# yukara-ikemiya/friendly-stable-audio-tools

Hardware: NVIDIA H100
Metric: denoise_steps_per_s (higher is better)
Workload: dtype fp16 operands, fp32 accumulate (the reference's autocast dtype)

## Files before the change

friendly-stable-audio-tools_b200/csrc/attention_tc.cu:

```cuda
#include "common.cuh"
#include "gemm.cuh"
#include "kernels.h"
#include "ptx.cuh"
#include <cmath>

namespace satb {

namespace {

constexpr int kQ = 64;
constexpr int kK = 64;
constexpr int kAttnThreads = 128;
template <int D>
constexpr int tile_elems() { return 64 * D; }
template <int D>
constexpr int attn_smem() { return (1 + 2 * 2) * tile_elems<D>() * 2; }

struct AttnArgs {
  const uint16_t *q, *k, *v;
  uint16_t* o;
  int64_t ldq, ldk, ldv, ldo, q_bs, k_bs, v_bs, o_bs;
  int q_col, k_col, v_col;
  int Nq, Nk, group;
  float scale_log2;
};

template <int D>
// ... 186 lines not shown
    l[i] += __shfl_xor_sync(0xffffffffu, l[i], 2);
    inv[i] = 1.f / l[i];
  }
  const int rr = warp * 16 + (lane >> 2);
#pragma unroll
  for (int j = 0; j < D / 8; ++j) {
    const int col = 8 * j + 2 * (lane & 3);
    *reinterpret_cast<uint32_t*>(sQ + swz<D>(rr, col >> 3) + (col & 7)) = Op16<BF16>::pack(o[j][0] * inv[0], o[j][1] * inv[0]);
    *reinterpret_cast<uint32_t*>(sQ + swz<D>(rr + 8, col >> 3) + (col & 7)) =
        Op16<BF16>::pack(o[j][2] * inv[1], o[j][3] * inv[1]);
  }
  __syncwarp();
  uint16_t* ob = p.o + b * p.o_bs + h * D;
#pragma unroll
  for (int i = 0; i < 16 * kChunks / 32; ++i) {
    const int idx = lane + 32 * i;
    const int r = warp * 16 + chunk_row<kChunks>(idx), c = chunk_col<kChunks>(idx);
    if (q0 + r < p.Nq)
      *reinterpret_cast<uint4*>(ob + static_cast<int64_t>(q0 + r) * p.ldo + c * 8) =
          *reinterpret_cast<const uint4*>(sQ + swz<D>(r, c));
  }
}

}

int launch_attention_tc(const void* q, const void* k, const void* v, void* o, int64_t ldq, int64_t ldk, int64_t ldv,
                        int64_t ldo, int64_t q_bs, int64_t k_bs, int64_t v_bs, int64_t o_bs, int q_cols, int k_cols,
                        int v_cols, int q_col, int k_col, int v_col, int batch, int H, int H_kv, int Nq, int Nk,
                        int head_dim, bool bf16, cudaStream_t stream) {
  SATB_REQUIRE(head_dim == 32 || head_dim == 64 || head_dim == 96 || head_dim == 128,
               "attention head dim must be 32, 64, 96 or 128");
  SATB_REQUIRE(H >= 1 && H_kv >= 1, "attention needs at least one head");
  SATB_REQUIRE(H % H_kv == 0, "num_heads must be a multiple of kv heads");
  SATB_REQUIRE(Nk >= 1 && Nq >= 1, "empty attention problem");
  SATB_REQUIRE(ldo % 8 == 0 && o_bs % 8 == 0 && (reinterpret_cast<uintptr_t>(o) & 15) == 0,
               "attention output must be 16B aligned");
  SATB_REQUIRE(ldq % 8 == 0 && ldk % 8 == 0 && ldv % 8 == 0 && q_col % 8 == 0 && k_col % 8 == 0 && v_col % 8 == 0 &&
                   q_bs % 8 == 0 && k_bs % 8 == 0 && v_bs % 8 == 0,
               "attention operand strides / column offsets must be 16B aligned");
  SATB_REQUIRE((reinterpret_cast<uintptr_t>(q) & 15) == 0 && (reinterpret_cast<uintptr_t>(k) & 15) == 0 &&
                   (reinterpret_cast<uintptr_t>(v) & 15) == 0,
               "attention operands must be 16B aligned");
  const int64_t dh = head_dim;
  SATB_REQUIRE(q_col + H * dh <= q_cols && k_col + H_kv * dh <= k_cols && v_col + H_kv * dh <= v_cols,
               "attention heads exceed the operand columns");
  AttnArgs a;
  a.q = static_cast<const uint16_t*>(q); a.k = static_cast<const uint16_t*>(k); a.v = static_cast<const uint16_t*>(v);
  a.o = static_cast<uint16_t*>(o);
  a.ldq = ldq; a.ldk = ldk; a.ldv = ldv; a.ldo = ldo;
  a.q_bs = q_bs; a.k_bs = k_bs; a.v_bs = v_bs; a.o_bs = o_bs;
  a.q_col = q_col; a.k_col = k_col; a.v_col = v_col;
  a.Nq = Nq; a.Nk = Nk; a.group = H / H_kv;
  a.scale_log2 = (1.0f / sqrtf(static_cast<float>(head_dim))) * 1.4426950408889634f;
  const dim3 grid(ceil_div(Nq, kQ), H, batch);
  SATB_REQUIRE(grid.y <= 65535 && grid.z <= 65535, "attention grid too large");
  auto go = [&](auto kern, int smem, PerDeviceOnce& once) -> int {
    if (once.first()) SATB_CHECK_CUDA(cudaFuncSetAttribute(kern, cudaFuncAttributeMaxDynamicSharedMemorySize, smem));
    SATB_CHECK_CUDA(launch_pdl(kern, grid, dim3(kAttnThreads), smem, stream, a));
    return 0;
  };
  static PerDeviceOnce once[4][2];
  PerDeviceOnce& on = once[head_dim / 32 - 1][bf16 ? 1 : 0];
  switch (head_dim) {
    case 32: SATB_PROPAGATE(bf16 ? go(attn_kernel<32, true>, attn_smem<32>(), on) : go(attn_kernel<32, false>, attn_smem<32>(), on)); break;
    case 64: SATB_PROPAGATE(bf16 ? go(attn_kernel<64, true>, attn_smem<64>(), on) : go(attn_kernel<64, false>, attn_smem<64>(), on)); break;
    case 96: SATB_PROPAGATE(bf16 ? go(attn_kernel<96, true>, attn_smem<96>(), on) : go(attn_kernel<96, false>, attn_smem<96>(), on)); break;
    default: SATB_PROPAGATE(bf16 ? go(attn_kernel<128, true>, attn_smem<128>(), on) : go(attn_kernel<128, false>, attn_smem<128>(), on)); break;
  }
  count_launch();
  SATB_CHECK_CUDA(cudaGetLastError());
  return 0;
}

}
```

friendly-stable-audio-tools_b200/csrc/dit.cu:

```cuda
#include <algorithm>
#include <cmath>
#include <cstring>
#include <map>
#include <string>
#include <tuple>
#include <vector>

#include "../../include/satb200.h"
#include "common.cuh"
#include "gemm.cuh"
#include "kernels.h"

namespace satb {

struct DevBuf {
  void* p = nullptr;
  size_t bytes = 0;
  int ensure(size_t need) {
    if (need <= bytes) return 0;
    if (p) cudaFree(p);
    p = nullptr;
    bytes = 0;
    cudaError_t e = cudaMalloc(&p, need);
    if (e != cudaSuccess) {
// ... 598 lines not shown
      SATB_PROPAGATE(launch_layernorm(h, W.pre_g, W.pre_b, a16, M, D, ssg_l, ssg_l ? ssg_l + D : nullptr, ssg_ld, N_seq, B, BF16, st));
    }
    {
      ProfScope ps(d, PROF_QKV, st);
      if (d->qk_norm) {
        typedef EpiHeadNorm16<BF16> E;
        typename E::Params ep{qkv, 3 * D, 2 * D, 2 * D, N_seq, cos_tab, sin_tab};
        SATB_PROPAGATE((linear<E, 256, BF16>(d->tmaps, a16, D, M, D, W.w_qkv, 3 * D, ep, st)));
      } else {
        if (fused && i > 0) {
          typedef EpiQkvRope<BF16, true> E;
          typename E::Params ep{qkv, 3 * D, 2 * D, N_seq, d->dh, d->nf, cos_tab, sin_tab, fold(S1, W.c_qkv, W.d_qkv)};
          SATB_PROPAGATE((linear<E, 256, BF16>(d->tmaps, a16, D, M, D, W.w_qkv, 3 * D, ep, st)));
        } else {
          typedef EpiQkvRope<BF16> E;
          typename E::Params ep{qkv, 3 * D, 2 * D, N_seq, d->dh, d->nf, cos_tab, sin_tab, no_ln};
          SATB_PROPAGATE((linear<E, 256, BF16>(d->tmaps, a16, D, M, D, W.w_qkv, 3 * D, ep, st)));
        }
      }
    }
    {
      ProfScope ps(d, PROF_ATTN_SELF, st);
      const int64_t qs = static_cast<int64_t>(N_seq) * 3 * D;
      SATB_PROPAGATE(launch_attention_tc(qkv, qkv, qkv, att, 3 * D, 3 * D, 3 * D, D, qs, qs, qs,
                                         static_cast<int64_t>(N_seq) * D, 3 * D, 3 * D, 3 * D, 0, D, 2 * D, R, H, H,
                                         N_seq, N_seq, d->dh, BF16, st));
    }
    {
      ProfScope ps(d, PROF_ATTN_OUT, st);
      if (fused) {
        typedef EpiResidualLN<BF16> E;
        typename E::Params ep{h, D, nullptr, a16, W.ca_g, W.ff_g, S2, S3, Mc};
        SATB_PROPAGATE((linear<E, 256, BF16>(d->tmaps, att, D, M, D, W.w_o, D, ep, st)));
      } else {
        EpiResidual::Params ep{h, D, nullptr, ssg_l ? ssg_l + 2 * D : nullptr, N_seq, static_cast<int>(ssg_ld), B};
        SATB_PROPAGATE((linear_auto<EpiResidual, BF16>(d->tmaps, att, D, M, D, W.w_o, D, ep, st)));
      }
    }
    if (Mc > 0) {
      ProfScope ps(d, PROF_CROSS, st);
      const int Hkv = d->ce / d->dh;
      if (!fused) SATB_PROPAGATE(launch_layernorm(h, W.ca_g, W.ca_b, a16, Mc, D, nullptr, nullptr, 0, N_seq, 1, BF16, st));
      if (d->qk_norm) {
        typedef EpiHeadNorm16<BF16> E;
        typename E::Params ep{q16, D, D, 0, N_seq, nullptr, nullptr};
        SATB_PROPAGATE((linear_auto<E, BF16>(d->tmaps, a16, D, Mc, D, W.w_q, D, ep, st)));
      } else {
        if (fused) {
          typedef EpiStore16<BF16, true> E;
          typename E::Params ep{q16, D, nullptr, 0, fold(S2, W.c_q, W.d_q)};
          SATB_PROPAGATE((linear_auto<E, BF16>(d->tmaps, a16, D, Mc, D, W.w_q, D, ep, st)));
        } else {
          typedef EpiStore16<BF16> E;
          typename E::Params ep{q16, D, nullptr, 0, no_ln};
          SATB_PROPAGATE((linear_auto<E, BF16>(d->tmaps, a16, D, Mc, D, W.w_q, D, ep, st)));
        }
      }
      const uint16_t* kv = d->ws_kv.as<uint16_t>() + static_cast<size_t>(i) * d->Rc * d->Mctx * 2 * d->ce;
      const int64_t kvs = static_cast<int64_t>(d->Mctx) * 2 * d->ce;
      SATB_PROPAGATE(launch_attention_tc(q16, kv, kv, att, D, 2 * d->ce, 2 * d->ce, D, static_cast<int64_t>(N_seq) * D,
                                         kvs, kvs, static_cast<int64_t>(N_seq) * D, D, 2 * d->ce, 2 * d->ce, 0, 0,
                                         d->ce, d->Rc, H, Hkv, N_seq, d->Mctx, d->dh, BF16, st));
      if (fused) {
        typedef EpiResidualLN<BF16> E;
        typename E::Params ep{h, D, nullptr, a16, W.ff_g, W.ff_g, S3, S3, Mc};
        SATB_PROPAGATE((linear<E, 256, BF16>(d->tmaps, att, D, Mc, D, W.w_co, D, ep, st)));
      } else {
        EpiResidual::Params ep{h, D, nullptr, nullptr, N_seq, 0, 1};
        SATB_PROPAGATE((linear_auto<EpiResidual, BF16>(d->tmaps, att, D, Mc, D, W.w_co, D, ep, st)));
      }
    }
    if (!fused) {
      ProfScope ps(d, PROF_LN, st);
      SATB_PROPAGATE(launch_layernorm(h, W.ff_g, W.ff_b, a16, M, D, ssg_l ? ssg_l + 3 * D : nullptr,
                                      ssg_l ? ssg_l + 4 * D : nullptr, ssg_ld, N_seq, B, BF16, st));
    }
    {
      ProfScope ps(d, PROF_FF_IN, st);
      if (fused) {
        typedef EpiSwiglu<BF16, true> E;
        typename E::Params ep{ff, d->ffi, W.b_ff1, fold(S3, W.c_ff1, W.d_ff1)};
        SATB_PROPAGATE((linear<E, 256, BF16>(d->tmaps, a16, D, M, D, W.w_ff1, 2 * d->ffi, ep, st)));
      } else {
        typedef EpiSwiglu<BF16> E;
        typename E::Params ep{ff, d->ffi, W.b_ff1, no_ln};
// ... 196 lines not shown
```

friendly-stable-audio-tools_b200/csrc/kernels.h:

```cpp
#pragma once
#include <cuda_runtime.h>
#include <stdint.h>

namespace satb {

int launch_attention_tc(const void* q, const void* k, const void* v, void* o, int64_t ldq, int64_t ldk, int64_t ldv,
                        int64_t ldo, int64_t q_bs, int64_t k_bs, int64_t v_bs, int64_t o_bs, int q_cols, int k_cols,
                        int v_cols, int q_col, int k_col, int v_col, int batch, int H, int H_kv, int Nq, int Nk,
                        int head_dim, bool bf16, cudaStream_t stream);
bool conv_halo_enabled();
bool resunit_use_fused();
bool conv_epi_masked();
bool ln_fold_enabled();
bool raw_stream_16bit();

int launch_layernorm(const float* x, const float* gamma, const float* beta, void* out16, int rows, int D,
                     const float* scale, const float* shift, int64_t mod_stride, int rows_per_item, int n_items,
                     bool bf16, cudaStream_t stream);
int launch_ln_fold_vectors(const void* w16, const float* gamma, const float* beta, float* c, float* d, int rows, int K,
                           bool bf16, cudaStream_t stream);
int launch_sampler_update(const float* x, const float* v, const float* d1, const float* d2, const float* nz, float* den,
                          float* x_next, float* x_in, long long n, float c_skip, float c_out, float A, float B, float C,
                          float D, float S, float c_in_next, cudaStream_t stream);
int launch_snake_beta(const float* x, const float* alpha, const float* beta, float* y, int B, int C, int64_t T,
                      int logscale, cudaStream_t stream);
int launch_dit_pre(const float* x, void* a16, int R, int B_src, int C, int L, int P, bool bf16, cudaStream_t stream);
int launch_fourier(const float* t, const float* w, float* out, int B, int F, cudaStream_t stream);
int launch_skinny_linear(const float* in, const float* W, const float* bias, const float* add, float* out, int R,
                         int K, int N, int silu_out, cudaStream_t stream);
int launch_write_prepend(const float* tok, const float* pre, float* h, int R, int B, int N_seq, int D, int Pp,
                         cudaStream_t stream);
int launch_gate_sigmoid(float* ssg, int rows, int depth, int D, cudaStream_t stream);
// ... 9 lines not shown
```

friendly-stable-audio-tools_b200/csrc/ptx.cuh:

```cuda
#pragma once
#include <cuda.h>
#include <cuda_runtime.h>
#include <stdint.h>

namespace satb {

__device__ __forceinline__ uint32_t smem_u32(const void* p) {
  return static_cast<uint32_t>(__cvta_generic_to_shared(p));
}

__device__ __forceinline__ bool elect_one() {
  uint32_t pred = 0;
  asm volatile(
      "{\n\t.reg .pred P;\n\t"
      "elect.sync _|P, 0xffffffff;\n\t"
      "selp.u32 %0, 1, 0, P;\n\t}"
      : "=r"(pred));
  return pred != 0;
}

__device__ __forceinline__ void pdl_wait() { asm volatile("griddepcontrol.wait;" ::: "memory"); }
__device__ __forceinline__ void pdl_launch_dependents() { asm volatile("griddepcontrol.launch_dependents;" ::: "memory"); }

__device__ __forceinline__ void mbar_init(uint64_t* bar, uint32_t count) {
// ... 142 lines not shown
template <>
__device__ __forceinline__ void wgmma_ss<256, false>(float (&d)[128], uint64_t da, uint64_t db, uint32_t accumulate) {
  asm volatile(
      "{\n\t.reg .pred p;\n\t"
      "setp.ne.b32 p, %130, 0;\n\t"
      "wgmma.mma_async.sync.aligned.m64n256k16.f32.f16.f16 "
      "{%0, %1, %2, %3, %4, %5, %6, %7, %8, %9, %10, %11, %12, %13, %14, %15, %16, %17, %18, %19, %20, %21, %22, %23, %24, %25, %26, %27, %28, %29, %30, %31, %32, %33, %34, %35, %36, %37, %38, %39, %40, %41, %42, %43, %44, %45, %46, %47, %48, %49, %50, %51, %52, %53, %54, %55, %56, %57, %58, %59, %60, %61, %62, %63, %64, %65, %66, %67, %68, %69, %70, %71, %72, %73, %74, %75, %76, %77, %78, %79, %80, %81, %82, %83, %84, %85, %86, %87, %88, %89, %90, %91, %92, %93, %94, %95, %96, %97, %98, %99, %100, %101, %102, %103, %104, %105, %106, %107, %108, %109, %110, %111, %112, %113, %114, %115, %116, %117, %118, %119, %120, %121, %122, %123, %124, %125, %126, %127}, "
      "%128, %129, p, 1, 1, 0, 0;\n\t}"
      : "+f"(d[0]), "+f"(d[1]), "+f"(d[2]), "+f"(d[3]), "+f"(d[4]), "+f"(d[5]), "+f"(d[6]), "+f"(d[7]), "+f"(d[8]), "+f"(d[9]), "+f"(d[10]), "+f"(d[11]), "+f"(d[12]), "+f"(d[13]), "+f"(d[14]), "+f"(d[15]), "+f"(d[16]), "+f"(d[17]), "+f"(d[18]), "+f"(d[19]), "+f"(d[20]), "+f"(d[21]), "+f"(d[22]), "+f"(d[23]), "+f"(d[24]), "+f"(d[25]), "+f"(d[26]), "+f"(d[27]), "+f"(d[28]), "+f"(d[29]), "+f"(d[30]), "+f"(d[31]), "+f"(d[32]), "+f"(d[33]), "+f"(d[34]), "+f"(d[35]), "+f"(d[36]), "+f"(d[37]), "+f"(d[38]), "+f"(d[39]), "+f"(d[40]), "+f"(d[41]), "+f"(d[42]), "+f"(d[43]), "+f"(d[44]), "+f"(d[45]), "+f"(d[46]), "+f"(d[47]), "+f"(d[48]), "+f"(d[49]), "+f"(d[50]), "+f"(d[51]), "+f"(d[52]), "+f"(d[53]), "+f"(d[54]), "+f"(d[55]), "+f"(d[56]), "+f"(d[57]), "+f"(d[58]), "+f"(d[59]), "+f"(d[60]), "+f"(d[61]), "+f"(d[62]), "+f"(d[63]), "+f"(d[64]), "+f"(d[65]), "+f"(d[66]), "+f"(d[67]), "+f"(d[68]), "+f"(d[69]), "+f"(d[70]), "+f"(d[71]), "+f"(d[72]), "+f"(d[73]), "+f"(d[74]), "+f"(d[75]), "+f"(d[76]), "+f"(d[77]), "+f"(d[78]), "+f"(d[79]), "+f"(d[80]), "+f"(d[81]), "+f"(d[82]), "+f"(d[83]), "+f"(d[84]), "+f"(d[85]), "+f"(d[86]), "+f"(d[87]), "+f"(d[88]), "+f"(d[89]), "+f"(d[90]), "+f"(d[91]), "+f"(d[92]), "+f"(d[93]), "+f"(d[94]), "+f"(d[95]), "+f"(d[96]), "+f"(d[97]), "+f"(d[98]), "+f"(d[99]), "+f"(d[100]), "+f"(d[101]), "+f"(d[102]), "+f"(d[103]), "+f"(d[104]), "+f"(d[105]), "+f"(d[106]), "+f"(d[107]), "+f"(d[108]), "+f"(d[109]), "+f"(d[110]), "+f"(d[111]), "+f"(d[112]), "+f"(d[113]), "+f"(d[114]), "+f"(d[115]), "+f"(d[116]), "+f"(d[117]), "+f"(d[118]), "+f"(d[119]), "+f"(d[120]), "+f"(d[121]), "+f"(d[122]), "+f"(d[123]), "+f"(d[124]), "+f"(d[125]), "+f"(d[126]), "+f"(d[127])
      : "l"(da), "l"(db), "r"(accumulate));
}
template <>
__device__ __forceinline__ void wgmma_ss<256, true>(float (&d)[128], uint64_t da, uint64_t db, uint32_t accumulate) {
  asm volatile(
      "{\n\t.reg .pred p;\n\t"
      "setp.ne.b32 p, %130, 0;\n\t"
      "wgmma.mma_async.sync.aligned.m64n256k16.f32.bf16.bf16 "
      "{%0, %1, %2, %3, %4, %5, %6, %7, %8, %9, %10, %11, %12, %13, %14, %15, %16, %17, %18, %19, %20, %21, %22, %23, %24, %25, %26, %27, %28, %29, %30, %31, %32, %33, %34, %35, %36, %37, %38, %39, %40, %41, %42, %43, %44, %45, %46, %47, %48, %49, %50, %51, %52, %53, %54, %55, %56, %57, %58, %59, %60, %61, %62, %63, %64, %65, %66, %67, %68, %69, %70, %71, %72, %73, %74, %75, %76, %77, %78, %79, %80, %81, %82, %83, %84, %85, %86, %87, %88, %89, %90, %91, %92, %93, %94, %95, %96, %97, %98, %99, %100, %101, %102, %103, %104, %105, %106, %107, %108, %109, %110, %111, %112, %113, %114, %115, %116, %117, %118, %119, %120, %121, %122, %123, %124, %125, %126, %127}, "
      "%128, %129, p, 1, 1, 0, 0;\n\t}"
      : "+f"(d[0]), "+f"(d[1]), "+f"(d[2]), "+f"(d[3]), "+f"(d[4]), "+f"(d[5]), "+f"(d[6]), "+f"(d[7]), "+f"(d[8]), "+f"(d[9]), "+f"(d[10]), "+f"(d[11]), "+f"(d[12]), "+f"(d[13]), "+f"(d[14]), "+f"(d[15]), "+f"(d[16]), "+f"(d[17]), "+f"(d[18]), "+f"(d[19]), "+f"(d[20]), "+f"(d[21]), "+f"(d[22]), "+f"(d[23]), "+f"(d[24]), "+f"(d[25]), "+f"(d[26]), "+f"(d[27]), "+f"(d[28]), "+f"(d[29]), "+f"(d[30]), "+f"(d[31]), "+f"(d[32]), "+f"(d[33]), "+f"(d[34]), "+f"(d[35]), "+f"(d[36]), "+f"(d[37]), "+f"(d[38]), "+f"(d[39]), "+f"(d[40]), "+f"(d[41]), "+f"(d[42]), "+f"(d[43]), "+f"(d[44]), "+f"(d[45]), "+f"(d[46]), "+f"(d[47]), "+f"(d[48]), "+f"(d[49]), "+f"(d[50]), "+f"(d[51]), "+f"(d[52]), "+f"(d[53]), "+f"(d[54]), "+f"(d[55]), "+f"(d[56]), "+f"(d[57]), "+f"(d[58]), "+f"(d[59]), "+f"(d[60]), "+f"(d[61]), "+f"(d[62]), "+f"(d[63]), "+f"(d[64]), "+f"(d[65]), "+f"(d[66]), "+f"(d[67]), "+f"(d[68]), "+f"(d[69]), "+f"(d[70]), "+f"(d[71]), "+f"(d[72]), "+f"(d[73]), "+f"(d[74]), "+f"(d[75]), "+f"(d[76]), "+f"(d[77]), "+f"(d[78]), "+f"(d[79]), "+f"(d[80]), "+f"(d[81]), "+f"(d[82]), "+f"(d[83]), "+f"(d[84]), "+f"(d[85]), "+f"(d[86]), "+f"(d[87]), "+f"(d[88]), "+f"(d[89]), "+f"(d[90]), "+f"(d[91]), "+f"(d[92]), "+f"(d[93]), "+f"(d[94]), "+f"(d[95]), "+f"(d[96]), "+f"(d[97]), "+f"(d[98]), "+f"(d[99]), "+f"(d[100]), "+f"(d[101]), "+f"(d[102]), "+f"(d[103]), "+f"(d[104]), "+f"(d[105]), "+f"(d[106]), "+f"(d[107]), "+f"(d[108]), "+f"(d[109]), "+f"(d[110]), "+f"(d[111]), "+f"(d[112]), "+f"(d[113]), "+f"(d[114]), "+f"(d[115]), "+f"(d[116]), "+f"(d[117]), "+f"(d[118]), "+f"(d[119]), "+f"(d[120]), "+f"(d[121]), "+f"(d[122]), "+f"(d[123]), "+f"(d[124]), "+f"(d[125]), "+f"(d[126]), "+f"(d[127])
      : "l"(da), "l"(db), "r"(accumulate));
}

template <int R>
__device__ __forceinline__ void setmaxnreg_dec() { asm volatile("setmaxnreg.dec.sync.aligned.u32 %0;" ::"n"(R)); }
template <int R>
__device__ __forceinline__ void setmaxnreg_inc() { asm volatile("setmaxnreg.inc.sync.aligned.u32 %0;" ::"n"(R)); }
__device__ __forceinline__ void named_bar_sync(int id, int count) {
  asm volatile("bar.sync %0, %1;" ::"r"(id), "r"(count) : "memory");
}

}
```

Baseline: 17.34.

## Add warp-specialized TMA+WGMMA flash attention kernel for head_dim 64

Adds a Hopper-style attention kernel for head_dim 64. One producer warpgroup loads Q/K/V tiles with TMA through a 4-stage mbarrier pipeline, and two consumer warpgroups run QK^T and PV with wgmma. The consumers ping-pong via named barriers so one warpgroup's softmax overlaps the other's matmul. Self- and cross-attention callers now pass cached tensor maps, and the old mma.sync 64-wide path is removed. This is meant to replace the previous cp.async/mma kernel with higher tensor-core throughput, at the cost of considerable new synchronization complexity and tail-tile specializations.

```diff
diff --git a/friendly-stable-audio-tools_b200/csrc/attention_tc.cu b/friendly-stable-audio-tools_b200/csrc/attention_tc.cu
--- a/friendly-stable-audio-tools_b200/csrc/attention_tc.cu
+++ b/friendly-stable-audio-tools_b200/csrc/attention_tc.cu
@@ -3,6 +3,7 @@
 #include "kernels.h"
 #include "ptx.cuh"
 #include <cmath>
+#include <type_traits>
 
 namespace satb {
 
@@ -235,12 +236,272 @@
   }
 }
 
+constexpr int kWgQ = 128;
+constexpr int kWgK = 128;
+constexpr int kWgStages = 4;
+constexpr int kWgThreads = 384;
+constexpr int kWgTile = 128 * 64 * 2;
+constexpr int kWgSmem = 1024  + kWgTile * (1 + 2 * kWgStages) + 256 ;
+constexpr int kBarTurn = 1;
+
+struct AttnWgArgs {
+  uint16_t* o;
+  int64_t ldo, o_bs;
+  int q_col, k_col, v_col;
+  int Nq, Nk, group;
+  float scale_log2;
+};
+
+template <int W, bool BF16>
+__device__ __forceinline__ void issue_qk(float (&s)[64], uint32_t q_addr, uint32_t k_addr) {
+#pragma unroll
+  for (int k = 0; k < 4; ++k)
+    wgmma_ss<W, BF16>(*reinterpret_cast<float(*)[W / 2]>(&s[0]), make_desc_kmajor_sw128(q_addr + 32 * k),
+                      make_desc_kmajor_sw128(k_addr + 32 * k), k != 0 ? 1u : 0u);
+}
+
+template <bool LAST>
+__device__ __forceinline__ void softmax_tile(float (&s)[64], float (&m)[2], float (&l)[2], float (&alpha)[2], float scale,
+                                             int w, int key0, int Nk) {
+  float mx[2] = {-INFINITY, -INFINITY};
+#pragma unroll
+  for (int g = 0; g < 16; ++g) {
+    if (LAST && 8 * g >= w) break;
+#pragma unroll
+    for (int e = 0; e < 4; ++e) {
+      if (LAST && key0 + 8 * g + (e & 1) >= Nk) s[4 * g + e] = -INFINITY;
+      mx[e >> 1] = fmaxf(mx[e >> 1], s[4 * g + e]);
+    }
+  }
+  float sum[2] = {0.f, 0.f};
+#pragma unroll
+  for (int i = 0; i < 2; ++i) {
+    mx[i] = fmaxf(mx[i], __shfl_xor_sync(0xffffffffu, mx[i], 1));
+    mx[i] = fmaxf(mx[i], __shfl_xor_sync(0xffffffffu, mx[i], 2));
+    const float mn = fmaxf(m[i], mx[i] * scale);
+    alpha[i] = exp2f(m[i] - mn);
+    m[i] = mn;
+  }
+#pragma unroll
+  for (int g = 0; g < 16; ++g) {
+    if (LAST && 8 * g >= w) break;
+#pragma unroll
+    for (int e = 0; e < 4; ++e) {
+      s[4 * g + e] = exp2f(fmaf(s[4 * g + e], scale, -m[e >> 1]));
+      sum[e >> 1] += s[4 * g + e];
+    }
+  }
+#pragma unroll
+  for (int i = 0; i < 2; ++i) l[i] = fmaf(l[i], alpha[i], sum[i]);
+}
+
+template <bool BF16>
+__global__ void __launch_bounds__(kWgThreads, 1)
+attn_wgmma_kernel(const __grid_constant__ CUtensorMap tmq, const __grid_constant__ CUtensorMap tmk,
+                  const __grid_constant__ CUtensorMap tmv, const AttnWgArgs p) {
+  extern __shared__ uint8_t smem_wg[];
+  uint8_t* sQ = reinterpret_cast<uint8_t*>((reinterpret_cast<uintptr_t>(smem_wg) + 1023) & ~uintptr_t(1023));
+  uint8_t* sK = sQ + kWgTile;
+  uint8_t* sV = sK + kWgStages * kWgTile;
+  uint64_t* q_bar = reinterpret_cast<uint64_t*>(sV + kWgStages * kWgTile);
+  uint64_t* full_bar = q_bar + 1;
+  uint64_t* empty_bar = full_bar + kWgStages;
+
+  const int warp = threadIdx.x >> 5, lane = threadIdx.x & 31;
+  const int wg = __shfl_sync(0xffffffffu, static_cast<int>(threadIdx.x >> 7), 0);
+  const int q0 = blockIdx.x * kWgQ, h = blockIdx.y, b = blockIdx.z;
+  const int n_tiles = (p.Nk + kWgK - 1) / kWgK;
+
+  if (threadIdx.x == 0) {
+    tma_prefetch_desc(&tmq);
+    tma_prefetch_desc(&tmk);
+    tma_prefetch_desc(&tmv);
+    mbar_init(q_bar, 1);
+    for (int i = 0; i < kWgStages; ++i) {
+      mbar_init(&full_bar[i], 1);
+      mbar_init(&empty_bar[i], 2);
+    }
+    fence_mbar_init();
+  }
+  __syncthreads();
+  pdl_launch_dependents();
+
+  if (wg == 0) {
+    setmaxnreg_dec<40>();
+    if (warp == 0 && elect_one()) {
+      pdl_wait();
+      const int hk = h / p.group;
+      mbar_expect_tx(q_bar, kWgTile);
+      tma_load_4d(sQ, &tmq, q_bar, p.q_col + h * 64, 0, q0, b);
+      for (int j = 0; j < n_tiles; ++j) {
+        const int st = j % kWgStages;
+        mbar_wait(&empty_bar[st], ((j / kWgStages) & 1) ^ 1);
+        mbar_expect_tx(&full_bar[st], 2 * kWgTile);
+        tma_load_4d(sK + st * kWgTile, &tmk, &full_bar[st], p.k_col + hk * 64, 0, j * kWgK, b);
+        tma_load_4d(sV + st * kWgTile, &tmv, &full_bar[st], p.v_col + hk * 64, 0, j * kWgK, b);
+      }
+    }
+  } else {
+    setmaxnreg_inc<232>();
+    pdl_wait();
+    const int cw = wg - 1;
+    const bool active = q0 + 64 * cw < p.Nq;
+    const uint32_t q_addr = smem_u32(sQ) + cw * 64 * 128;
+    const int rem = p.Nk - (n_tiles - 1) * kWgK;
+    const int w_last = (rem + 15) & ~15;
+    const int key_lane = 2 * (lane & 3);
+
+    if (!active) {
+      if (cw == 1) named_bar_arrive(kBarTurn, 256);
+      for (int j = 0; j <= n_tiles; ++j) {
+        named_bar_sync(kBarTurn + cw, 256);
+        if (cw == 0 || j < n_tiles) named_bar_arrive(kBarTurn + (cw ^ 1), 256);
+        if (j > 0 && (threadIdx.x & 127) == 0) mbar_arrive(&empty_bar[(j - 1) % kWgStages]);
+      }
+      return;
+    }
+
+    float s[64], o[32];
+    uint32_t pf[8][4];
+    float m[2] = {-1e30f, -1e30f}, l[2] = {0.f, 0.f}, alpha[2];
+#pragma unroll
+    for (int i = 0; i < 64; ++i) s[i] = 0.f;
+#pragma unroll
+    for (int i = 0; i < 32; ++i) o[i] = 0.f;
+
+    auto issue_pv = [&](int j, int w) {
+      const uint32_t v_addr = smem_u32(sV + (j % kWgStages) * kWgTile);
+#pragma unroll
+      for (int kk = 0; kk < 8; ++kk)
+        if (16 * kk < w) wgmma_rs_tb<64, BF16>(o, pf[kk], make_desc_mnmajor_sw128(v_addr + 2048 * kk), 1u);
+    };
+    auto retire_pv = [&](int j) {
+      wgmma_wait<0>(o);
+#pragma unroll
+      for (int kk = 0; kk < 8; ++kk) wgmma_fence_regs(pf[kk]);
+      if ((threadIdx.x & 127) == 0) mbar_arrive(&empty_bar[j % kWgStages]);
+    };
+    auto rescale_and_pack = [&](int w) {
+#pragma unroll
+      for (int g = 0; g < 8; ++g) {
+        o[4 * g] *= alpha[0];
+        o[4 * g + 1] *= alpha[0];
+        o[4 * g + 2] *= alpha[1];
+        o[4 * g + 3] *= alpha[1];
+      }
+#pragma unroll
+      for (int kk = 0; kk < 8; ++kk) {
+        if (16 * kk >= w) break;
+        pf[kk][0] = Op16<BF16>::pack(s[8 * kk], s[8 * kk + 1]);
+        pf[kk][1] = Op16<BF16>::pack(s[8 * kk + 2], s[8 * kk + 3]);
+        pf[kk][2] = Op16<BF16>::pack(s[8 * kk + 4], s[8 * kk + 5]);
+        pf[kk][3] = Op16<BF16>::pack(s[8 * kk + 6], s[8 * kk + 7]);
+      }
+    };
+    auto full_turn = [&](int j, auto prevc) {
+      constexpr bool PREV = decltype(prevc)::value;
+      mbar_wait(&full_bar[j % kWgStages], (j / kWgStages) & 1);
+      named_bar_sync(kBarTurn + cw, 256);
+      wgmma_fence();
+      issue_qk<kWgK, BF16>(s, q_addr, smem_u32(sK + (j % kWgStages) * kWgTile));
+      wgmma_commit();
+      if constexpr (PREV) {
+        issue_pv(j - 1, kWgK);
+        wgmma_commit();
+      }
+      named_bar_arrive(kBarTurn + (cw ^ 1), 256);
+      if constexpr (PREV) wgmma_wait<1>(s);
+      else wgmma_wait<0>(s);
+      softmax_tile<false>(s, m, l, alpha, p.scale_log2, kWgK, j * kWgK + key_lane, p.Nk);
+      if constexpr (PREV) retire_pv(j - 1);
+      rescale_and_pack(kWgK);
+    };
+    auto last_turns = [&](auto wc, auto prevc) {
+      constexpr int W = decltype(wc)::value;
+      constexpr bool PREV = decltype(prevc)::value;
+      const int j = n_tiles - 1;
+      mbar_wait(&full_bar[j % kWgStages], (j / kWgStages) & 1);
+      named_bar_sync(kBarTurn + cw, 256);
+      wgmma_fence();
+      issue_qk<W, BF16>(s, q_addr, smem_u32(sK + (j % kWgStages) * kWgTile));
+      wgmma_commit();
+      if constexpr (PREV) {
+        issue_pv(j - 1, kWgK);
+        wgmma_commit();
+      }
+      named_bar_arrive(kBarTurn + (cw ^ 1), 256);
+      if constexpr (PREV) wgmma_wait<1>(s);
+      else wgmma_wait<0>(s);
+      softmax_tile<true>(s, m, l, alpha, p.scale_log2, W, j * kWgK + key_lane, p.Nk);
+      if constexpr (PREV) retire_pv(j - 1);
+      rescale_and_pack(W);
+      named_bar_sync(kBarTurn + cw, 256);
+      wgmma_fence();
+      issue_pv(j, W);
+      wgmma_commit();
+      if (cw == 0) named_bar_arrive(kBarTurn + 1, 256);
+      retire_pv(j);
+    };
+    auto last_turns_w = [&](auto prevc) {
+      switch (w_last) {
+        case 16: last_turns(std::integral_constant<int, 16>{}, prevc); break;
+        case 32: last_turns(std::integral_constant<int, 32>{}, prevc); break;
+        case 48: last_turns(std::integral_constant<int, 48>{}, prevc); break;
+        case 64: last_turns(std::integral_constant<int, 64>{}, prevc); break;
+        case 80: last_turns(std::integral_constant<int, 80>{}, prevc); break;
+        case 96: last_turns(std::integral_constant<int, 96>{}, prevc); break;
+        case 112: last_turns(std::integral_constant<int, 112>{}, prevc); break;
+        default: last_turns(std::integral_constant<int, 128>{}, prevc); break;
+      }
+    };
+
+    mbar_wait(q_bar, 0);
+    if (cw == 1) named_bar_arrive(kBarTurn, 256);
+    if (n_tiles == 1) {
+      last_turns_w(std::false_type{});
+    } else {
+      full_turn(0, std::false_type{});
+      for (int j = 1; j < n_tiles - 1; ++j) full_turn(j, std::true_type{});
+      last_turns_w(std::true_type{});
+    }
+
+    float inv[2];
+#pragma unroll
+    for (int i = 0; i < 2; ++i) {
+      l[i] += __shfl_xor_sync(0xffffffffu, l[i], 1);
+      l[i] += __shfl_xor_sync(0xffffffffu, l[i], 2);
+      inv[i] = 1.f / l[i];
+    }
+    uint16_t* so = reinterpret_cast<uint16_t*>(sQ + cw * 64 * 128);
+    const int wq = warp & 3;
+    const int rr = 16 * wq + (lane >> 2);
+#pragma unroll
+    for (int g = 0; g < 8; ++g) {
+      *reinterpret_cast<uint32_t*>(so + swz<64>(rr, g) + key_lane) = Op16<BF16>::pack(o[4 * g] * inv[0], o[4 * g + 1] * inv[0]);
+      *reinterpret_cast<uint32_t*>(so + swz<64>(rr + 8, g) + key_lane) =
+          Op16<BF16>::pack(o[4 * g + 2] * inv[1], o[4 * g + 3] * inv[1]);
+    }
+    __syncwarp();
+    uint16_t* ob = p.o + b * p.o_bs + h * 64;
+#pragma unroll
+    for (int i = 0; i < 4; ++i) {
+      const int idx = lane + 32 * i;
+      const int r = 16 * wq + (idx >> 3), c = idx & 7;
+      const int row = q0 + 64 * cw + r;
+      if (row < p.Nq)
+        *reinterpret_cast<uint4*>(ob + static_cast<int64_t>(row) * p.ldo + c * 8) =
+            *reinterpret_cast<const uint4*>(so + swz<64>(r, c));
+    }
+  }
+}
+
 }
 
 int launch_attention_tc(const void* q, const void* k, const void* v, void* o, int64_t ldq, int64_t ldk, int64_t ldv,
                         int64_t ldo, int64_t q_bs, int64_t k_bs, int64_t v_bs, int64_t o_bs, int q_cols, int k_cols,
                         int v_cols, int q_col, int k_col, int v_col, int batch, int H, int H_kv, int Nq, int Nk,
-                        int head_dim, bool bf16, cudaStream_t stream) {
+                        int head_dim, bool bf16, cudaStream_t stream, const CUtensorMap* tmq, const CUtensorMap* tmk,
+                        const CUtensorMap* tmv) {
   SATB_REQUIRE(head_dim == 32 || head_dim == 64 || head_dim == 96 || head_dim == 128,
                "attention head dim must be 32, 64, 96 or 128");
   SATB_REQUIRE(H >= 1 && H_kv >= 1, "attention needs at least one head");
@@ -265,6 +526,28 @@
   a.q_col = q_col; a.k_col = k_col; a.v_col = v_col;
   a.Nq = Nq; a.Nk = Nk; a.group = H / H_kv;
   a.scale_log2 = (1.0f / sqrtf(static_cast<float>(head_dim))) * 1.4426950408889634f;
+  if (head_dim == 64) {
+    CUtensorMap mq, mk, mv;
+    if (!tmq) SATB_PROPAGATE(make_tmap_a(&mq, q, q_cols, Nq, batch, ldq, q_bs));
+    if (!tmk) SATB_PROPAGATE(make_tmap_a(&mk, k, k_cols, Nk, batch, ldk, k_bs));
+    if (!tmv) SATB_PROPAGATE(make_tmap_a(&mv, v, v_cols, Nk, batch, ldv, v_bs));
+    AttnWgArgs w;
+    w.o = a.o; w.ldo = ldo; w.o_bs = o_bs;
+    w.q_col = q_col; w.k_col = k_col; w.v_col = v_col;
+    w.Nq = Nq; w.Nk = Nk; w.group = a.group;
+    w.scale_log2 = a.scale_log2;
+    const dim3 grid(ceil_div(Nq, kWgQ), H, batch);
+    SATB_REQUIRE(grid.y <= 65535 && grid.z <= 65535, "attention grid too large");
+    auto kern = bf16 ? attn_wgmma_kernel<true> : attn_wgmma_kernel<false>;
+    static PerDeviceOnce once_wg[2];
+    if (once_wg[bf16 ? 1 : 0].first())
+      SATB_CHECK_CUDA(cudaFuncSetAttribute(kern, cudaFuncAttributeMaxDynamicSharedMemorySize, kWgSmem));
+    SATB_CHECK_CUDA(launch_pdl(kern, grid, dim3(kWgThreads), kWgSmem, stream, tmq ? *tmq : mq, tmk ? *tmk : mk,
+                               tmv ? *tmv : mv, w));
+    count_launch();
+    SATB_CHECK_CUDA(cudaGetLastError());
+    return 0;
+  }
   const dim3 grid(ceil_div(Nq, kQ), H, batch);
   SATB_REQUIRE(grid.y <= 65535 && grid.z <= 65535, "attention grid too large");
   auto go = [&](auto kern, int smem, PerDeviceOnce& once) -> int {
@@ -276,7 +559,6 @@
   PerDeviceOnce& on = once[head_dim / 32 - 1][bf16 ? 1 : 0];
   switch (head_dim) {
     case 32: SATB_PROPAGATE(bf16 ? go(attn_kernel<32, true>, attn_smem<32>(), on) : go(attn_kernel<32, false>, attn_smem<32>(), on)); break;
-    case 64: SATB_PROPAGATE(bf16 ? go(attn_kernel<64, true>, attn_smem<64>(), on) : go(attn_kernel<64, false>, attn_smem<64>(), on)); break;
     case 96: SATB_PROPAGATE(bf16 ? go(attn_kernel<96, true>, attn_smem<96>(), on) : go(attn_kernel<96, false>, attn_smem<96>(), on)); break;
     default: SATB_PROPAGATE(bf16 ? go(attn_kernel<128, true>, attn_smem<128>(), on) : go(attn_kernel<128, false>, attn_smem<128>(), on)); break;
   }
diff --git a/friendly-stable-audio-tools_b200/csrc/dit.cu b/friendly-stable-audio-tools_b200/csrc/dit.cu
--- a/friendly-stable-audio-tools_b200/csrc/dit.cu
+++ b/friendly-stable-audio-tools_b200/csrc/dit.cu
@@ -644,9 +644,11 @@
     {
       ProfScope ps(d, PROF_ATTN_SELF, st);
       const int64_t qs = static_cast<int64_t>(N_seq) * 3 * D;
+      const CUtensorMap* tm = nullptr;
+      if (d->dh == 64) SATB_PROPAGATE(d->tmaps.get_a(qkv, 3 * D, N_seq, R, 3 * D, qs, &tm));
       SATB_PROPAGATE(launch_attention_tc(qkv, qkv, qkv, att, 3 * D, 3 * D, 3 * D, D, qs, qs, qs,
                                          static_cast<int64_t>(N_seq) * D, 3 * D, 3 * D, 3 * D, 0, D, 2 * D, R, H, H,
-                                         N_seq, N_seq, d->dh, BF16, st));
+                                         N_seq, N_seq, d->dh, BF16, st, tm, tm, tm));
     }
     {
       ProfScope ps(d, PROF_ATTN_OUT, st);
@@ -680,9 +682,14 @@
       }
       const uint16_t* kv = d->ws_kv.as<uint16_t>() + static_cast<size_t>(i) * d->Rc * d->Mctx * 2 * d->ce;
       const int64_t kvs = static_cast<int64_t>(d->Mctx) * 2 * d->ce;
+      const CUtensorMap *tq = nullptr, *tkv = nullptr;
+      if (d->dh == 64) {
+        SATB_PROPAGATE(d->tmaps.get_a(q16, D, N_seq, d->Rc, D, static_cast<int64_t>(N_seq) * D, &tq));
+        SATB_PROPAGATE(d->tmaps.get_a(kv, 2 * d->ce, d->Mctx, d->Rc, 2 * d->ce, kvs, &tkv));
+      }
       SATB_PROPAGATE(launch_attention_tc(q16, kv, kv, att, D, 2 * d->ce, 2 * d->ce, D, static_cast<int64_t>(N_seq) * D,
                                          kvs, kvs, static_cast<int64_t>(N_seq) * D, D, 2 * d->ce, 2 * d->ce, 0, 0,
-                                         d->ce, d->Rc, H, Hkv, N_seq, d->Mctx, d->dh, BF16, st));
+                                         d->ce, d->Rc, H, Hkv, N_seq, d->Mctx, d->dh, BF16, st, tq, tkv, tkv));
       if (fused) {
         typedef EpiResidualLN<BF16> E;
         typename E::Params ep{h, D, nullptr, a16, W.ff_g, W.ff_g, S3, S3, Mc};
diff --git a/friendly-stable-audio-tools_b200/csrc/kernels.h b/friendly-stable-audio-tools_b200/csrc/kernels.h
--- a/friendly-stable-audio-tools_b200/csrc/kernels.h
+++ b/friendly-stable-audio-tools_b200/csrc/kernels.h
@@ -1,4 +1,5 @@
 #pragma once
+#include <cuda.h>
 #include <cuda_runtime.h>
 #include <stdint.h>
 
@@ -7,7 +8,8 @@
 int launch_attention_tc(const void* q, const void* k, const void* v, void* o, int64_t ldq, int64_t ldk, int64_t ldv,
                         int64_t ldo, int64_t q_bs, int64_t k_bs, int64_t v_bs, int64_t o_bs, int q_cols, int k_cols,
                         int v_cols, int q_col, int k_col, int v_col, int batch, int H, int H_kv, int Nq, int Nk,
-                        int head_dim, bool bf16, cudaStream_t stream);
+                        int head_dim, bool bf16, cudaStream_t stream, const CUtensorMap* tmq = nullptr,
+                        const CUtensorMap* tmk = nullptr, const CUtensorMap* tmv = nullptr);
 bool conv_halo_enabled();
 bool resunit_use_fused();
 bool conv_epi_masked();
diff --git a/friendly-stable-audio-tools_b200/csrc/ptx.cuh b/friendly-stable-audio-tools_b200/csrc/ptx.cuh
--- a/friendly-stable-audio-tools_b200/csrc/ptx.cuh
+++ b/friendly-stable-audio-tools_b200/csrc/ptx.cuh
@@ -188,6 +188,178 @@
       : "l"(da), "l"(db), "r"(accumulate));
 }
 
+template <>
+__device__ __forceinline__ void wgmma_ss<16, false>(float (&d)[8], uint64_t da, uint64_t db, uint32_t accumulate) {
+  asm volatile(
+      "{\n\t.reg .pred p;\n\t"
+      "setp.ne.b32 p, %10, 0;\n\t"
+      "wgmma.mma_async.sync.aligned.m64n16k16.f32.f16.f16 "
+      "{%0, %1, %2, %3, %4, %5, %6, %7}, "
+      "%8, %9, p, 1, 1, 0, 0;\n\t}"
+      : "+f"(d[0]), "+f"(d[1]), "+f"(d[2]), "+f"(d[3]), "+f"(d[4]), "+f"(d[5]), "+f"(d[6]), "+f"(d[7])
+      : "l"(da), "l"(db), "r"(accumulate));
+}
+template <>
+__device__ __forceinline__ void wgmma_ss<16, true>(float (&d)[8], uint64_t da, uint64_t db, uint32_t accumulate) {
+  asm volatile(
+      "{\n\t.reg .pred p;\n\t"
+      "setp.ne.b32 p, %10, 0;\n\t"
+      "wgmma.mma_async.sync.aligned.m64n16k16.f32.bf16.bf16 "
+      "{%0, %1, %2, %3, %4, %5, %6, %7}, "
+      "%8, %9, p, 1, 1, 0, 0;\n\t}"
+      : "+f"(d[0]), "+f"(d[1]), "+f"(d[2]), "+f"(d[3]), "+f"(d[4]), "+f"(d[5]), "+f"(d[6]), "+f"(d[7])
+      : "l"(da), "l"(db), "r"(accumulate));
+}
+template <>
+__device__ __forceinline__ void wgmma_ss<32, false>(float (&d)[16], uint64_t da, uint64_t db, uint32_t accumulate) {
+  asm volatile(
+      "{\n\t.reg .pred p;\n\t"
+      "setp.ne.b32 p, %18, 0;\n\t"
+      "wgmma.mma_async.sync.aligned.m64n32k16.f32.f16.f16 "
+      "{%0, %1, %2, %3, %4, %5, %6, %7, %8, %9, %10, %11, %12, %13, %14, %15}, "
+      "%16, %17, p, 1, 1, 0, 0;\n\t}"
+      : "+f"(d[0]), "+f"(d[1]), "+f"(d[2]), "+f"(d[3]), "+f"(d[4]), "+f"(d[5]), "+f"(d[6]), "+f"(d[7]), "+f"(d[8]), "+f"(d[9]), "+f"(d[10]), "+f"(d[11]), "+f"(d[12]), "+f"(d[13]), "+f"(d[14]), "+f"(d[15])
+      : "l"(da), "l"(db), "r"(accumulate));
+}
+template <>
+__device__ __forceinline__ void wgmma_ss<32, true>(float (&d)[16], uint64_t da, uint64_t db, uint32_t accumulate) {
+  asm volatile(
+      "{\n\t.reg .pred p;\n\t"
+      "setp.ne.b32 p, %18, 0;\n\t"
+      "wgmma.mma_async.sync.aligned.m64n32k16.f32.bf16.bf16 "
+      "{%0, %1, %2, %3, %4, %5, %6, %7, %8, %9, %10, %11, %12, %13, %14, %15}, "
+      "%16, %17, p, 1, 1, 0, 0;\n\t}"
+      : "+f"(d[0]), "+f"(d[1]), "+f"(d[2]), "+f"(d[3]), "+f"(d[4]), "+f"(d[5]), "+f"(d[6]), "+f"(d[7]), "+f"(d[8]), "+f"(d[9]), "+f"(d[10]), "+f"(d[11]), "+f"(d[12]), "+f"(d[13]), "+f"(d[14]), "+f"(d[15])
+      : "l"(da), "l"(db), "r"(accumulate));
+}
+template <>
+__device__ __forceinline__ void wgmma_ss<48, false>(float (&d)[24], uint64_t da, uint64_t db, uint32_t accumulate) {
+  asm volatile(
+      "{\n\t.reg .pred p;\n\t"
+      "setp.ne.b32 p, %26, 0;\n\t"
+      "wgmma.mma_async.sync.aligned.m64n48k16.f32.f16.f16 "
+      "{%0, %1, %2, %3, %4, %5, %6, %7, %8, %9, %10, %11, %12, %13, %14, %15, %16, %17, %18, %19, %20, %21, %22, %23}, "
+      "%24, %25, p, 1, 1, 0, 0;\n\t}"
+      : "+f"(d[0]), "+f"(d[1]), "+f"(d[2]), "+f"(d[3]), "+f"(d[4]), "+f"(d[5]), "+f"(d[6]), "+f"(d[7]), "+f"(d[8]), "+f"(d[9]), "+f"(d[10]), "+f"(d[11]), "+f"(d[12]), "+f"(d[13]), "+f"(d[14]), "+f"(d[15]), "+f"(d[16]), "+f"(d[17]), "+f"(d[18]), "+f"(d[19]), "+f"(d[20]), "+f"(d[21]), "+f"(d[22]), "+f"(d[23])
+      : "l"(da), "l"(db), "r"(accumulate));
+}
+template <>
+__device__ __forceinline__ void wgmma_ss<48, true>(float (&d)[24], uint64_t da, uint64_t db, uint32_t accumulate) {
+  asm volatile(
+      "{\n\t.reg .pred p;\n\t"
+      "setp.ne.b32 p, %26, 0;\n\t"
+      "wgmma.mma_async.sync.aligned.m64n48k16.f32.bf16.bf16 "
+      "{%0, %1, %2, %3, %4, %5, %6, %7, %8, %9, %10, %11, %12, %13, %14, %15, %16, %17, %18, %19, %20, %21, %22, %23}, "
+      "%24, %25, p, 1, 1, 0, 0;\n\t}"
+      : "+f"(d[0]), "+f"(d[1]), "+f"(d[2]), "+f"(d[3]), "+f"(d[4]), "+f"(d[5]), "+f"(d[6]), "+f"(d[7]), "+f"(d[8]), "+f"(d[9]), "+f"(d[10]), "+f"(d[11]), "+f"(d[12]), "+f"(d[13]), "+f"(d[14]), "+f"(d[15]), "+f"(d[16]), "+f"(d[17]), "+f"(d[18]), "+f"(d[19]), "+f"(d[20]), "+f"(d[21]), "+f"(d[22]), "+f"(d[23])
+      : "l"(da), "l"(db), "r"(accumulate));
+}
+template <>
+__device__ __forceinline__ void wgmma_ss<80, false>(float (&d)[40], uint64_t da, uint64_t db, uint32_t accumulate) {
+  asm volatile(
+      "{\n\t.reg .pred p;\n\t"
+      "setp.ne.b32 p, %42, 0;\n\t"
+      "wgmma.mma_async.sync.aligned.m64n80k16.f32.f16.f16 "
+      "{%0, %1, %2, %3, %4, %5, %6, %7, %8, %9, %10, %11, %12, %13, %14, %15, %16, %17, %18, %19, %20, %21, %22, %23, %24, %25, %26, %27, %28, %29, %30, %31, %32, %33, %34, %35, %36, %37, %38, %39}, "
+      "%40, %41, p, 1, 1, 0, 0;\n\t}"
+      : "+f"(d[0]), "+f"(d[1]), "+f"(d[2]), "+f"(d[3]), "+f"(d[4]), "+f"(d[5]), "+f"(d[6]), "+f"(d[7]), "+f"(d[8]), "+f"(d[9]), "+f"(d[10]), "+f"(d[11]), "+f"(d[12]), "+f"(d[13]), "+f"(d[14]), "+f"(d[15]), "+f"(d[16]), "+f"(d[17]), "+f"(d[18]), "+f"(d[19]), "+f"(d[20]), "+f"(d[21]), "+f"(d[22]), "+f"(d[23]), "+f"(d[24]), "+f"(d[25]), "+f"(d[26]), "+f"(d[27]), "+f"(d[28]), "+f"(d[29]), "+f"(d[30]), "+f"(d[31]), "+f"(d[32]), "+f"(d[33]), "+f"(d[34]), "+f"(d[35]), "+f"(d[36]), "+f"(d[37]), "+f"(d[38]), "+f"(d[39])
+      : "l"(da), "l"(db), "r"(accumulate));
+}
+template <>
+__device__ __forceinline__ void wgmma_ss<80, true>(float (&d)[40], uint64_t da, uint64_t db, uint32_t accumulate) {
+  asm volatile(
+      "{\n\t.reg .pred p;\n\t"
+      "setp.ne.b32 p, %42, 0;\n\t"
+      "wgmma.mma_async.sync.aligned.m64n80k16.f32.bf16.bf16 "
+      "{%0, %1, %2, %3, %4, %5, %6, %7, %8, %9, %10, %11, %12, %13, %14, %15, %16, %17, %18, %19, %20, %21, %22, %23, %24, %25, %26, %27, %28, %29, %30, %31, %32, %33, %34, %35, %36, %37, %38, %39}, "
+      "%40, %41, p, 1, 1, 0, 0;\n\t}"
+      : "+f"(d[0]), "+f"(d[1]), "+f"(d[2]), "+f"(d[3]), "+f"(d[4]), "+f"(d[5]), "+f"(d[6]), "+f"(d[7]), "+f"(d[8]), "+f"(d[9]), "+f"(d[10]), "+f"(d[11]), "+f"(d[12]), "+f"(d[13]), "+f"(d[14]), "+f"(d[15]), "+f"(d[16]), "+f"(d[17]), "+f"(d[18]), "+f"(d[19]), "+f"(d[20]), "+f"(d[21]), "+f"(d[22]), "+f"(d[23]), "+f"(d[24]), "+f"(d[25]), "+f"(d[26]), "+f"(d[27]), "+f"(d[28]), "+f"(d[29]), "+f"(d[30]), "+f"(d[31]), "+f"(d[32]), "+f"(d[33]), "+f"(d[34]), "+f"(d[35]), "+f"(d[36]), "+f"(d[37]), "+f"(d[38]), "+f"(d[39])
+      : "l"(da), "l"(db), "r"(accumulate));
+}
+template <>
+__device__ __forceinline__ void wgmma_ss<96, false>(float (&d)[48], uint64_t da, uint64_t db, uint32_t accumulate) {
+  asm volatile(
+      "{\n\t.reg .pred p;\n\t"
+      "setp.ne.b32 p, %50, 0;\n\t"
+      "wgmma.mma_async.sync.aligned.m64n96k16.f32.f16.f16 "
+      "{%0, %1, %2, %3, %4, %5, %6, %7, %8, %9, %10, %11, %12, %13, %14, %15, %16, %17, %18, %19, %20, %21, %22, %23, %24, %25, %26, %27, %28, %29, %30, %31, %32, %33, %34, %35, %36, %37, %38, %39, %40, %41, %42, %43, %44, %45, %46, %47}, "
+      "%48, %49, p, 1, 1, 0, 0;\n\t}"
+      : "+f"(d[0]), "+f"(d[1]), "+f"(d[2]), "+f"(d[3]), "+f"(d[4]), "+f"(d[5]), "+f"(d[6]), "+f"(d[7]), "+f"(d[8]), "+f"(d[9]), "+f"(d[10]), "+f"(d[11]), "+f"(d[12]), "+f"(d[13]), "+f"(d[14]), "+f"(d[15]), "+f"(d[16]), "+f"(d[17]), "+f"(d[18]), "+f"(d[19]), "+f"(d[20]), "+f"(d[21]), "+f"(d[22]), "+f"(d[23]), "+f"(d[24]), "+f"(d[25]), "+f"(d[26]), "+f"(d[27]), "+f"(d[28]), "+f"(d[29]), "+f"(d[30]), "+f"(d[31]), "+f"(d[32]), "+f"(d[33]), "+f"(d[34]), "+f"(d[35]), "+f"(d[36]), "+f"(d[37]), "+f"(d[38]), "+f"(d[39]), "+f"(d[40]), "+f"(d[41]), "+f"(d[42]), "+f"(d[43]), "+f"(d[44]), "+f"(d[45]), "+f"(d[46]), "+f"(d[47])
+      : "l"(da), "l"(db), "r"(accumulate));
+}
+template <>
+__device__ __forceinline__ void wgmma_ss<96, true>(float (&d)[48], uint64_t da, uint64_t db, uint32_t accumulate) {
+  asm volatile(
+      "{\n\t.reg .pred p;\n\t"
+      "setp.ne.b32 p, %50, 0;\n\t"
+      "wgmma.mma_async.sync.aligned.m64n96k16.f32.bf16.bf16 "
+      "{%0, %1, %2, %3, %4, %5, %6, %7, %8, %9, %10, %11, %12, %13, %14, %15, %16, %17, %18, %19, %20, %21, %22, %23, %24, %25, %26, %27, %28, %29, %30, %31, %32, %33, %34, %35, %36, %37, %38, %39, %40, %41, %42, %43, %44, %45, %46, %47}, "
+      "%48, %49, p, 1, 1, 0, 0;\n\t}"
+      : "+f"(d[0]), "+f"(d[1]), "+f"(d[2]), "+f"(d[3]), "+f"(d[4]), "+f"(d[5]), "+f"(d[6]), "+f"(d[7]), "+f"(d[8]), "+f"(d[9]), "+f"(d[10]), "+f"(d[11]), "+f"(d[12]), "+f"(d[13]), "+f"(d[14]), "+f"(d[15]), "+f"(d[16]), "+f"(d[17]), "+f"(d[18]), "+f"(d[19]), "+f"(d[20]), "+f"(d[21]), "+f"(d[22]), "+f"(d[23]), "+f"(d[24]), "+f"(d[25]), "+f"(d[26]), "+f"(d[27]), "+f"(d[28]), "+f"(d[29]), "+f"(d[30]), "+f"(d[31]), "+f"(d[32]), "+f"(d[33]), "+f"(d[34]), "+f"(d[35]), "+f"(d[36]), "+f"(d[37]), "+f"(d[38]), "+f"(d[39]), "+f"(d[40]), "+f"(d[41]), "+f"(d[42]), "+f"(d[43]), "+f"(d[44]), "+f"(d[45]), "+f"(d[46]), "+f"(d[47])
+      : "l"(da), "l"(db), "r"(accumulate));
+}
+template <>
+__device__ __forceinline__ void wgmma_ss<112, false>(float (&d)[56], uint64_t da, uint64_t db, uint32_t accumulate) {
+  asm volatile(
+      "{\n\t.reg .pred p;\n\t"
+      "setp.ne.b32 p, %58, 0;\n\t"
+      "wgmma.mma_async.sync.aligned.m64n112k16.f32.f16.f16 "
+      "{%0, %1, %2, %3, %4, %5, %6, %7, %8, %9, %10, %11, %12, %13, %14, %15, %16, %17, %18, %19, %20, %21, %22, %23, %24, %25, %26, %27, %28, %29, %30, %31, %32, %33, %34, %35, %36, %37, %38, %39, %40, %41, %42, %43, %44, %45, %46, %47, %48, %49, %50, %51, %52, %53, %54, %55}, "
+      "%56, %57, p, 1, 1, 0, 0;\n\t}"
+      : "+f"(d[0]), "+f"(d[1]), "+f"(d[2]), "+f"(d[3]), "+f"(d[4]), "+f"(d[5]), "+f"(d[6]), "+f"(d[7]), "+f"(d[8]), "+f"(d[9]), "+f"(d[10]), "+f"(d[11]), "+f"(d[12]), "+f"(d[13]), "+f"(d[14]), "+f"(d[15]), "+f"(d[16]), "+f"(d[17]), "+f"(d[18]), "+f"(d[19]), "+f"(d[20]), "+f"(d[21]), "+f"(d[22]), "+f"(d[23]), "+f"(d[24]), "+f"(d[25]), "+f"(d[26]), "+f"(d[27]), "+f"(d[28]), "+f"(d[29]), "+f"(d[30]), "+f"(d[31]), "+f"(d[32]), "+f"(d[33]), "+f"(d[34]), "+f"(d[35]), "+f"(d[36]), "+f"(d[37]), "+f"(d[38]), "+f"(d[39]), "+f"(d[40]), "+f"(d[41]), "+f"(d[42]), "+f"(d[43]), "+f"(d[44]), "+f"(d[45]), "+f"(d[46]), "+f"(d[47]), "+f"(d[48]), "+f"(d[49]), "+f"(d[50]), "+f"(d[51]), "+f"(d[52]), "+f"(d[53]), "+f"(d[54]), "+f"(d[55])
+      : "l"(da), "l"(db), "r"(accumulate));
+}
+template <>
+__device__ __forceinline__ void wgmma_ss<112, true>(float (&d)[56], uint64_t da, uint64_t db, uint32_t accumulate) {
+  asm volatile(
+      "{\n\t.reg .pred p;\n\t"
+      "setp.ne.b32 p, %58, 0;\n\t"
+      "wgmma.mma_async.sync.aligned.m64n112k16.f32.bf16.bf16 "
+      "{%0, %1, %2, %3, %4, %5, %6, %7, %8, %9, %10, %11, %12, %13, %14, %15, %16, %17, %18, %19, %20, %21, %22, %23, %24, %25, %26, %27, %28, %29, %30, %31, %32, %33, %34, %35, %36, %37, %38, %39, %40, %41, %42, %43, %44, %45, %46, %47, %48, %49, %50, %51, %52, %53, %54, %55}, "
+      "%56, %57, p, 1, 1, 0, 0;\n\t}"
+      : "+f"(d[0]), "+f"(d[1]), "+f"(d[2]), "+f"(d[3]), "+f"(d[4]), "+f"(d[5]), "+f"(d[6]), "+f"(d[7]), "+f"(d[8]), "+f"(d[9]), "+f"(d[10]), "+f"(d[11]), "+f"(d[12]), "+f"(d[13]), "+f"(d[14]), "+f"(d[15]), "+f"(d[16]), "+f"(d[17]), "+f"(d[18]), "+f"(d[19]), "+f"(d[20]), "+f"(d[21]), "+f"(d[22]), "+f"(d[23]), "+f"(d[24]), "+f"(d[25]), "+f"(d[26]), "+f"(d[27]), "+f"(d[28]), "+f"(d[29]), "+f"(d[30]), "+f"(d[31]), "+f"(d[32]), "+f"(d[33]), "+f"(d[34]), "+f"(d[35]), "+f"(d[36]), "+f"(d[37]), "+f"(d[38]), "+f"(d[39]), "+f"(d[40]), "+f"(d[41]), "+f"(d[42]), "+f"(d[43]), "+f"(d[44]), "+f"(d[45]), "+f"(d[46]), "+f"(d[47]), "+f"(d[48]), "+f"(d[49]), "+f"(d[50]), "+f"(d[51]), "+f"(d[52]), "+f"(d[53]), "+f"(d[54]), "+f"(d[55])
+      : "l"(da), "l"(db), "r"(accumulate));
+}
+__device__ __forceinline__ uint64_t make_desc_mnmajor_sw128(uint32_t smem_addr) {
+  uint64_t d = 0;
+  d |= static_cast<uint64_t>((smem_addr >> 4) & 0x3FFF);
+  d |= static_cast<uint64_t>(1) << 16;
+  d |= static_cast<uint64_t>(1024 >> 4) << 32;
+  d |= static_cast<uint64_t>(1) << 62;
+  return d;
+}
+template <int R>
+__device__ __forceinline__ void wgmma_fence_regs(uint32_t (&a)[R]) {
+#pragma unroll
+  for (int i = 0; i < R; ++i) asm volatile("" : "+r"(a[i])::"memory");
+}
+template <int N, bool BF16>
+__device__ __forceinline__ void wgmma_rs_tb(float (&d)[N / 2], const uint32_t (&a)[4], uint64_t db, uint32_t accumulate);
+template <>
+__device__ __forceinline__ void wgmma_rs_tb<64, false>(float (&d)[32], const uint32_t (&a)[4], uint64_t db,
+                                                        uint32_t accumulate) {
+  asm volatile(
+      "{\n\t.reg .pred p;\n\t"
+      "setp.ne.b32 p, %37, 0;\n\t"
+      "wgmma.mma_async.sync.aligned.m64n64k16.f32.f16.f16 "
+      "{%0, %1, %2, %3, %4, %5, %6, %7, %8, %9, %10, %11, %12, %13, %14, %15, %16, %17, %18, %19, %20, %21, %22, %23, %24, %25, %26, %27, %28, %29, %30, %31}, "
+      "{%32, %33, %34, %35}, %36, p, 1, 1, 1;\n\t}"
+      : "+f"(d[0]), "+f"(d[1]), "+f"(d[2]), "+f"(d[3]), "+f"(d[4]), "+f"(d[5]), "+f"(d[6]), "+f"(d[7]), "+f"(d[8]), "+f"(d[9]), "+f"(d[10]), "+f"(d[11]), "+f"(d[12]), "+f"(d[13]), "+f"(d[14]), "+f"(d[15]), "+f"(d[16]), "+f"(d[17]), "+f"(d[18]), "+f"(d[19]), "+f"(d[20]), "+f"(d[21]), "+f"(d[22]), "+f"(d[23]), "+f"(d[24]), "+f"(d[25]), "+f"(d[26]), "+f"(d[27]), "+f"(d[28]), "+f"(d[29]), "+f"(d[30]), "+f"(d[31])
+      : "r"(a[0]), "r"(a[1]), "r"(a[2]), "r"(a[3]), "l"(db), "r"(accumulate));
+}
+template <>
+__device__ __forceinline__ void wgmma_rs_tb<64, true>(float (&d)[32], const uint32_t (&a)[4], uint64_t db,
+                                                        uint32_t accumulate) {
+  asm volatile(
+      "{\n\t.reg .pred p;\n\t"
+      "setp.ne.b32 p, %37, 0;\n\t"
+      "wgmma.mma_async.sync.aligned.m64n64k16.f32.bf16.bf16 "
+      "{%0, %1, %2, %3, %4, %5, %6, %7, %8, %9, %10, %11, %12, %13, %14, %15, %16, %17, %18, %19, %20, %21, %22, %23, %24, %25, %26, %27, %28, %29, %30, %31}, "
+      "{%32, %33, %34, %35}, %36, p, 1, 1, 1;\n\t}"
+      : "+f"(d[0]), "+f"(d[1]), "+f"(d[2]), "+f"(d[3]), "+f"(d[4]), "+f"(d[5]), "+f"(d[6]), "+f"(d[7]), "+f"(d[8]), "+f"(d[9]), "+f"(d[10]), "+f"(d[11]), "+f"(d[12]), "+f"(d[13]), "+f"(d[14]), "+f"(d[15]), "+f"(d[16]), "+f"(d[17]), "+f"(d[18]), "+f"(d[19]), "+f"(d[20]), "+f"(d[21]), "+f"(d[22]), "+f"(d[23]), "+f"(d[24]), "+f"(d[25]), "+f"(d[26]), "+f"(d[27]), "+f"(d[28]), "+f"(d[29]), "+f"(d[30]), "+f"(d[31])
+      : "r"(a[0]), "r"(a[1]), "r"(a[2]), "r"(a[3]), "l"(db), "r"(accumulate));
+}
+
 template <int R>
 __device__ __forceinline__ void setmaxnreg_dec() { asm volatile("setmaxnreg.dec.sync.aligned.u32 %0;" ::"n"(R)); }
 template <int R>
@@ -195,5 +367,8 @@
 __device__ __forceinline__ void named_bar_sync(int id, int count) {
   asm volatile("bar.sync %0, %1;" ::"r"(id), "r"(count) : "memory");
 }
-
-}
+__device__ __forceinline__ void named_bar_arrive(int id, int count) {
+  asm volatile("bar.arrive %0, %1;" ::"r"(id), "r"(count) : "memory");
+}
+
+}
```

After: 18.51, median of 6. 1.07x the previous value.
